# ChaissonLab/LRA

Measured on AMD Instinct MI355X. Metric: aligned Gbp/s, 30 kb ONT vs GRCh38 (MapRead_lowacc end to end incl. SAM text), per job, higher is better.
Workload: dtype int32

## Files before the change

### lra_amd/csrc/common.h

```cpp
#pragma once
#include <hip/hip_runtime.h>
#include <stdint.h>
#include <stdio.h>
#include <atomic>
#include <memory>
#include <string>
#include <string.h>
#include <vector>
#include "../../include/lra_hip.h"

struct lra_seed_state;
struct lra_cluster_state;
struct lra_map_state;
struct lra_handover;
void lra_handover_free(lra_ctx* ctx);
struct lra_gen_cell { std::atomic<uint64_t> gen{0}; std::atomic<bool> dead{false}; };
struct lra_time_rec { const char* name; hipEvent_t a, b; hipStream_t stream; };

struct lra_ctx {
  int device = 0;
  hipStream_t stream = nullptr;
  std::string err;
  void* scratch[4] = {nullptr, nullptr, nullptr, nullptr};
  size_t scratch_bytes[4] = {0, 0, 0, 0};
  int num_cu = 256;
  lra_seed_state* seed = nullptr;
  lra_cluster_state* clus = nullptr;
  lra_map_state* map = nullptr;
  void* aux = nullptr; size_t aux_bytes = 0;
  void* out_buf = nullptr; size_t out_bytes = 0;
  void* pin_buf = nullptr; size_t pin_bytes = 0;
  void* rec_pin = nullptr; size_t rec_pin_bytes = 0;
  void* sv_pin = nullptr; size_t sv_pin_bytes = 0;
  void* bgzf_pin = nullptr; size_t bgzf_pin_bytes = 0;
  std::vector<uint64_t> bgzf_member_off;
  int bgzf_round = 0;
  double bgzf_ms = 0; uint64_t bgzf_bytes = 0;
  void* bam_buf[6] = {}; size_t bam_bytes[6] = {};
  int bam_cigar_limit = 65535;
  uint64_t* scan_tmp = nullptr;
  static constexpr int N_SIDE = 4;
  hipStream_t side[N_SIDE] = {}; hipEvent_t ev_fork = nullptr, ev_join[N_SIDE] = {}, ev_mid = nullptr;
  void* gbuf[192] = {};
  size_t gbytes[192] = {};
  bool sdp_inner = false;
  bool timing = false;
  std::vector<lra_time_rec> recs;
  std::vector<hipEvent_t> free_events;
  lra_ctx* child = nullptr;
  bool owns_stream = false;
  bool pipelined = false;
  struct lra_handover* handover = nullptr;
  struct { bool valid = false; int n_reads = 0; const char* d_seq = nullptr; const uint64_t* d_read_off = nullptr; int k = 0, w = 0, max_freq = 0; lra_seed_result res; } ahead;
  bool store_all = false;
  int svsig_len = 25;
  bool low_priority = false; int prio = 0;
};

hipStream_t lra_side_fork(lra_ctx* ctx, int i = 0);
void lra_side_join(lra_ctx* ctx, int i = 0);
hipError_t lra_segsort_pairs(lra_ctx* ctx, void* temp, size_t& temp_bytes, const uint64_t* kin, uint64_t* kout, const uint32_t* vin, uint32_t* vout, unsigned int total,
                             unsigned int nseg, const uint64_t* b, const uint64_t* e, int begin_bit, int end_bit, hipStream_t st);
int lra_segsort_pairs_scratch(lra_ctx* ctx, const uint64_t* kin, uint64_t* kout, const uint32_t* vin, uint32_t* vout, uint64_t total, uint64_t nseg, const uint64_t* b,
                              const uint64_t* e, int begin_bit, int end_bit);
void lra_time_begin(lra_ctx* ctx, const char* name, hipStream_t stream = nullptr);
void lra_time_end(lra_ctx* ctx, hipStream_t stream = nullptr);
void lra_seed_free(lra_ctx* ctx);
void lra_cluster_free(lra_ctx* ctx);
void lra_map_free(lra_ctx* ctx);

int lra_set_err(lra_ctx* ctx, int code, const char* fmt, ...);
int lra_host_threads();
void* lra_scratch(lra_ctx* ctx, int slot, size_t bytes);
void* lra_pinned(lra_ctx* ctx, size_t bytes);
void* lra_ensure(lra_ctx* ctx, int idx, size_t bytes);

struct lra_sort_opts { const char* tag = "sort"; const char* fb_tag = "sort_fallback"; bool short_lists = false; };
int lra_sort_exact_batch(lra_ctx* ctx, int n_lists, const uint64_t* d_off, uint64_t* d_key, uint32_t* d_pos, const lra_sort_opts& o = lra_sort_opts(),
                         const int* only = nullptr);
int lra_sort_mostly_unique_batch(lra_ctx* ctx, int n_lists, const uint64_t* d_off, uint64_t total, uint64_t* d_key, uint32_t* d_pos,
                                 uint64_t* tmp_key, uint32_t* tmp_pos, int end_bit, const lra_sort_opts& o = lra_sort_opts());

int lra_launch_linear_extend(lra_ctx* ctx, uint64_t n_clusters, int K, const uint64_t* c_start, const uint64_t* c_end, const int* c_strand, const int* c_chrom,
                             int* c_read, const uint32_t* cl_q, const uint32_t* cl_t, const uint64_t* d_chrom_pos, const unsigned char* genome,
                             const unsigned char* seq, const uint64_t* read_off, uint32_t* e_q, uint32_t* e_t, int* e_len, uint32_t* e_count, uint32_t* box,
                             const int* c_K = nullptr);

int lra_format_bed_str(const lra_aln_record* r, std::string& s_);
int lra_format_paf_str(const lra_aln_record* r, int print_cigar, std::string& s_);
int lra_format_sam_str(const lra_aln_record* g, int n_group, int as, int hard_clip, const char* passthrough, std::string& s_);
int lra_format_sam_simple_str(const lra_aln_record* rp, int hard_clip, const char* passthrough, std::string& s_);
int lra_output_read_str(const lra_aln_group* groups, const int32_t* index, int n_groups, lra_aln_record* recs, int print_num_aln, char format, int hard_clip,
                        const char* passthrough, int read_unaligned, const lra_aln_record* unaligned_rec, std::string& text);

#define LRA_HIP_CHECK(ctx, call)                                                         \
  do {                                                                                   \
    hipError_t e__ = (call);                                                             \
    if (e__ != hipSuccess)                                                               \
      return lra_set_err(ctx, LRA_ERR_HIP, "%s failed: %s (%s:%d)", #call,               \
                         hipGetErrorString(e__), __FILE__, __LINE__);                    \
  } while (0)
```

### lra_amd/csrc/exact_sort.hip

```cpp
#include "common.h"
#include "kmer.h"
#include "std_sort.h"
#include <algorithm>

namespace {

constexpr int SORT_CAP = 9000;

struct MaskedLess {
  template <class V> __host__ __device__ __forceinline__ bool operator()(const V& a, const V& b) const { return (a.k & KM_FOR_MASK) < (b.k & KM_FOR_MASK); }
};

__global__ void __launch_bounds__(64) sort_kernel(int n_reads, const uint64_t* __restrict__ mm_off, uint64_t* mm_key, uint32_t* mm_pos,
                                                  const int* __restrict__ only_flagged) {
  const int r = blockIdx.x * 64 + threadIdx.x;
  if (r >= n_reads) return;
  if (only_flagged && !only_flagged[r]) return;
  lra_std_sort::std_sort(lra_std_sort::Pairs<uint32_t>{mm_key + mm_off[r], mm_pos + mm_off[r]}, (long)(mm_off[r + 1] - mm_off[r]), MaskedLess());
}

constexpr int SORT_NT = 1024;
constexpr int SORT_NW = SORT_NT / 64;

template <int MODE> struct SortTypes { typedef unsigned short IT; typedef uint32_t TT; };
template <> struct SortTypes<2> { typedef uint32_t IT; typedef uint64_t TT; };
__host__ __device__ inline size_t sort_scratch_bytes(int mode, size_t cap) {
  const size_t isz = mode == 2 ? 4 : 2, maxseg = (cap / 16 + 8 + 1) & ~(size_t)1;
  size_t b = cap * 8 + 4 * cap * isz + 64;
  if (mode == 2) b += 10 * maxseg * isz + (cap / 32 + 2) * 4 + 64;
  return (b + 255) & ~(size_t)255;
}
template <int MODE>
__global__ void __launch_bounds__(SORT_NT) sort_wg_kernel(int n_reads, const uint64_t* __restrict__ mm_off, uint64_t* mm_key, uint32_t* mm_pos,
                                                        void* tscratch, int cap, int* __restrict__ fallback,
                                                        const int* __restrict__ only, char* gscr, int* stat, int minLen = 0) {
  constexpr bool BIG = MODE >= 1, HUGE = MODE == 2;
  typedef typename SortTypes<MODE>::IT IT;
  typedef typename SortTypes<MODE>::TT TT;
  constexpr IT S_NONE = (IT)~(IT)0;
  constexpr int HB = HUGE ? 32 : 16;
  constexpr TT HM = (TT)(((TT)1 << HB) - 1);
  extern __shared__ __attribute__((aligned(16))) char smem[];
  const int tid = threadIdx.x, lane = tid & 63, wave = tid >> 6;
  const int NT_ = (int)blockDim.x, NW_ = NT_ >> 6;
  const int maxseg = (cap / 16 + 8 + 1) & ~1;
  char* ebase = BIG ? gscr + (size_t)blockIdx.x * sort_scratch_bytes(MODE, (size_t)cap) : smem;
  uint64_t* key = (uint64_t*)ebase;
  IT* idx = (IT*)(key + cap);
  IT* seg = idx + cap;
  IT* pa = seg + cap;
  IT* pb = pa + cap;
  IT* sF = HUGE ? pb + cap : BIG ? (IT*)smem : pb + cap;
  IT* sL = sF + maxseg;
  IT* sD = sL + maxseg;
  IT* nF = sD + maxseg;
  IT* nL = nF + maxseg;
  IT* nD = nL + maxseg;
  IT* sCut = nD + maxseg;
  IT* sLid = sCut + maxseg;
  IT* sRid = sLid + maxseg;
  IT* sM = sRid + maxseg;
  unsigned int* startBits = (unsigned int*)(sM + maxseg + (maxseg & 1));
  __shared__ int cnt[4];
  __shared__ unsigned int waveTot[2 * SORT_NW];
  TT* t32 = (TT*)tscratch + (size_t)blockIdx.x * (size_t)(cap + 64);
  const lra_std_sort::Pairs<IT> S{key, idx};
  const MaskedLess lt;
  for (int r = blockIdx.x; r < n_reads; r += gridDim.x) {
    const long base = (long)mm_off[r];
    const int n = (int)(mm_off[r + 1] - mm_off[r]);
    if (n < 2) continue;
    if (BIG) {
      if (!fallback[r]) continue;
      if (n > cap) { if (MODE == 1 && stat && tid == 0) { atomicMax(&stat[0], n); atomicAdd(&stat[1], 1); } continue; }
    } else {
      if (only && !only[r]) continue;
      if (n < minLen) continue;
      if (n > cap) { if (fallback && tid == 0) { fallback[r] = 1; if (stat) atomicAdd(&stat[2], 1); } continue; }
    }
    __syncthreads();
    if (BIG && tid == 0) fallback[r] = 0;
    for (int p = tid; p < n; p += NT_) { key[p] = mm_key[base + p]; idx[p] = (IT)p; seg[p] = 0; }
    for (int x = tid; x < cap / 32 + 1; x += NT_) startBits[x] = 0;
    if (tid == 0) {
      if (n > 16) { sF[0] = 0; sL[0] = (IT)n; sD[0] = (IT)(2 * (31 - __clz(n))); cnt[0] = 1; }
      else cnt[0] = 0;
      cnt[1] = 0;
    }
    __syncthreads();
    if (tid == 0) startBits[0] = 1u;
    int nseg = cnt[0];
    while (nseg > 0) {
      for (int s = tid; s < nseg; s += NT_) {
        const int first = (int)sF[s], last = (int)sL[s];
        sM[s] = 0;
        if (sD[s] == 0) { lra_std_sort::heap_sort(S, first, last, lt); sM[s] = S_NONE; continue; }
        sD[s] = sD[s] - 1;
        lra_std_sort::move_median_to_first(S, first, last, lt);
      }
      __syncthreads();
      const int rows = (n + 63) / 64, rpw = (rows + NW_ - 1) / NW_;
      const int r0 = wave * rpw, r1 = min(rows, r0 + rpw);
      auto flags = [&](int p, bool& A, bool& B) {
        A = false; B = false;
        if (p < n) {
          const IT sg = seg[p];
          if (sg != S_NONE && sM[sg] != S_NONE && p != (int)sF[sg]) {
            const uint64_t piv = key[sF[sg]] & KM_FOR_MASK, km = key[p] & KM_FOR_MASK;
            A = km >= piv; B = km <= piv;
          }
        }
      };
      unsigned int totA = 0, totB = 0;
      for (int rw = r0; rw < r1; rw++) {
        bool A, B; flags(rw * 64 + lane, A, B);
        totA += __popcll(__ballot(A)); totB += __popcll(__ballot(B));
      }
      if (lane == 0) { waveTot[wave] = totA; waveTot[NW_ + wave] = totB; }
      __syncthreads();
      unsigned int baseA = 0, baseB = 0;
      for (int w = 0; w < wave; w++) { baseA += waveTot[w]; baseB += waveTot[NW_ + w]; }
      const unsigned long long below = (lane == 0) ? 0ULL : (~0ULL >> (64 - lane));
      for (int rw = r0; rw < r1; rw++) {
        const int p = rw * 64 + lane;
        bool A, B; flags(p, A, B);
        const unsigned long long mA = __ballot(A), mB = __ballot(B);
        if (p <= n) t32[p] = ((TT)(baseA + __popcll(mA & below)) & HM) | ((TT)(baseB + __popcll(mB & below)) << HB);
        baseA += __popcll(mA); baseB += __popcll(mB);
      }
      if (wave == NW_ - 1 && lane == 0 && (n & 63) == 0) t32[n] = ((TT)baseA & HM) | ((TT)baseB << HB);
      __syncthreads();
      for (int p = tid; p < n; p += NT_) {
        bool A, B; flags(p, A, B);
        if (A || B) {
          const int sg = (int)seg[p], b0 = (int)sF[sg] + 1;
          const TT t = t32[p], tb = t32[b0], te = t32[sL[sg]];
          if (A) pa[b0 + (int)(((t & HM) - (tb & HM)) & HM)] = (IT)p;
          if (B) pb[b0 + (int)(((te >> HB) - (t >> HB) - 1) & HM)] = (IT)p;
        }
      }
      __syncthreads();
      for (int p = tid; p < n; p += NT_) {
        const IT sg = seg[p];
        if (sg == S_NONE || sM[sg] == S_NONE) continue;
        const int b0 = (int)sF[sg] + 1, i = p - b0;
        if (i < 0) continue;
        const TT tb = t32[b0], te = t32[sL[sg]];
        const int nA = (int)(((te & HM) - (tb & HM)) & HM), nB = (int)(((te >> HB) - (tb >> HB)) & HM);
        const int lim = min(nA, nB);
        if (i < lim && pa[b0 + i] < pb[b0 + i] && !(i + 1 < lim && pa[b0 + i + 1] < pb[b0 + i + 1])) sM[sg] = (IT)(i + 1);
      }
      __syncthreads();
      for (int p = tid; p < n; p += NT_) {
        const IT sg = seg[p];
        if (sg == S_NONE || sM[sg] == S_NONE) continue;
        const int b0 = (int)sF[sg] + 1, i = p - b0;
        if (i >= 0 && i < (int)sM[sg]) lra_std_sort::iter_swap(S, (int)pa[b0 + i], (int)pb[b0 + i]);
      }
      __syncthreads();
      for (int s = tid; s < nseg; s += NT_) {
        const int first = (int)sF[s], last = (int)sL[s];
        if (sM[s] == S_NONE) { sCut[s] = (IT)last; sLid[s] = S_NONE; sRid[s] = S_NONE; continue; }
        const int b0 = first + 1, m = (int)sM[s];
        const TT tb = t32[b0], te = t32[last];
        const int nA = (int)(((te & HM) - (tb & HM)) & HM);
        int cut = 0x7fffffff;
        if (m < nA) cut = pa[b0 + m];
        if (m >= 1) cut = min(cut, (int)pb[b0 + m - 1]);
        sCut[s] = (IT)cut;
        IT lid = S_NONE, rid = S_NONE;
        if (cut - first > 16) { int x = atomicAdd(&cnt[1], 1); nF[x] = (IT)first; nL[x] = (IT)cut; nD[x] = sD[s]; lid = (IT)x; }
        if (last - cut > 16) { int x = atomicAdd(&cnt[1], 1); nF[x] = (IT)cut; nL[x] = (IT)last; nD[x] = sD[s]; rid = (IT)x; }
        atomicOr(&startBits[cut >> 5], 1u << (cut & 31));
        sLid[s] = lid; sRid[s] = rid;
      }
      __syncthreads();
      for (int p = tid; p < n; p += NT_) {
        const IT sg = seg[p];
        if (sg != S_NONE) seg[p] = (p < (int)sCut[sg]) ? sLid[sg] : sRid[sg];
      }
      nseg = cnt[1];
      __syncthreads();
      for (int s = tid; s < nseg; s += NT_) { sF[s] = nF[s]; sL[s] = nL[s]; sD[s] = nD[s]; }
      if (tid == 0) cnt[1] = 0;
      __syncthreads();
    }
    for (int p = tid; p < n; p += NT_) {
      if ((startBits[p >> 5] >> (p & 31)) & 1u) {
        int q = p + 1;
        while (q < n && !((startBits[q >> 5] >> (q & 31)) & 1u)) q++;
        lra_std_sort::insertion_sort(S, p, q, lt);
      }
    }
    __syncthreads();
    uint32_t* tmp = HUGE ? (uint32_t*)seg : (uint32_t*)pa;
    for (int p = tid; p < n; p += NT_) tmp[p] = mm_pos[base + idx[p]];
    __syncthreads();
    for (int p = tid; p < n; p += NT_) { mm_key[base + p] = key[p]; mm_pos[base + p] = tmp[p]; }
  }
}

}

int lra_sort_exact_batch(lra_ctx* ctx, int n_reads, const uint64_t* mm_off, uint64_t* mm_key, uint32_t* mm_pos, const lra_sort_opts& o, const int* only) {
  hipStream_t st = ctx->stream;
  const int nb = (n_reads + 63) / 64;
  const int cap = SORT_CAP, capB = 65534;
  const int maxseg = (cap / 16 + 8 + 1) & ~1, maxsegB = (capB / 16 + 8 + 1) & ~1;
  const size_t lds = (size_t)cap * 16 + (size_t)maxseg * 20 + 8 + (size_t)(cap / 32 + 2) * 4;
  const size_t ldsB = (size_t)maxsegB * 20 + 8 + (size_t)(capB / 32 + 2) * 4 + 64;
  const int grid = n_reads < ctx->num_cu ? n_reads : ctx->num_cu;
  const int gridB = std::min(grid, 64);
  const size_t tszB = (size_t)gridB * (capB + 64) * 4, esz = (size_t)gridB * sort_scratch_bytes(1, (size_t)capB);
  uint32_t* tscr = (uint32_t*)lra_scratch(ctx, 0, (size_t)grid * (cap + 64) * 4 + (size_t)n_reads * 4);
  char* big = (char*)lra_ensure(ctx, 85, tszB + esz + 1024);
  int* stat = (int*)lra_ensure(ctx, 97, 64);
  if (!tscr || !big || !stat) return LRA_ERR_NOMEM;
  uint32_t* tscrB = (uint32_t*)big; char* gscr = big + tszB;
  int* flags = (int*)(tscr + (size_t)grid * (cap + 64));
  LRA_HIP_CHECK(ctx, hipMemsetAsync(flags, 0, (size_t)n_reads * 4, st));
  LRA_HIP_CHECK(ctx, hipMemsetAsync(stat, 0, 12, st));
  LRA_HIP_CHECK(ctx, hipFuncSetAttribute((const void*)sort_wg_kernel<0>, hipFuncAttributeMaxDynamicSharedMemorySize, (int)lds));
  LRA_HIP_CHECK(ctx, hipFuncSetAttribute((const void*)sort_wg_kernel<1>, hipFuncAttributeMaxDynamicSharedMemorySize, (int)ldsB));
  lra_time_begin(ctx, o.tag);
  constexpr int capS = 2048;
  if (o.short_lists) {
    const int maxsegS = (capS / 16 + 8 + 1) & ~1;
    const size_t ldsS = (size_t)capS * 16 + (size_t)maxsegS * 20 + 8 + (size_t)(capS / 32 + 2) * 4;
    const int gridS = std::min(n_reads, std::min(ctx->num_cu * 4, (int)(((size_t)grid * (cap + 64)) / (size_t)(capS + 64))));
    hipLaunchKernelGGL(sort_wg_kernel<0>, dim3(gridS), dim3(256), ldsS, st, n_reads, mm_off, mm_key, mm_pos, (void*)tscr, capS, (int*)nullptr, only, (char*)nullptr, (int*)nullptr, 0);
  }
  hipLaunchKernelGGL(sort_wg_kernel<0>, dim3(grid), dim3(SORT_NT), lds, st, n_reads, mm_off, mm_key, mm_pos, (void*)tscr, cap, flags, only, (char*)nullptr, stat, o.short_lists ? capS + 1 : 0);
  lra_time_end(ctx);
  int h_left = 1;
  LRA_HIP_CHECK(ctx, hipMemcpyAsync(&h_left, stat + 2, 4, hipMemcpyDeviceToHost, st));
  LRA_HIP_CHECK(ctx, hipStreamSynchronize(st));
  if (h_left == 0) return LRA_OK;
  lra_time_begin(ctx, o.tag);
  hipLaunchKernelGGL(sort_wg_kernel<1>, dim3(gridB), dim3(SORT_NT), ldsB, st, n_reads, mm_off, mm_key, mm_pos, (void*)tscrB, capB, flags, only, gscr, stat);
  lra_time_end(ctx);
  int h_stat[2] = {0, 0};
  LRA_HIP_CHECK(ctx, hipMemcpyAsync(h_stat, stat, 8, hipMemcpyDeviceToHost, st));
  LRA_HIP_CHECK(ctx, hipStreamSynchronize(st));
  if (h_stat[1] == 0) return LRA_OK;
  const int capH = std::min(h_stat[0] + 64, (1 << 26));
  const int gridH = std::min(h_stat[1], std::max(1, ctx->num_cu));
  const size_t eszH = sort_scratch_bytes(2, (size_t)capH), tszH = (size_t)(capH + 64) * 8;
  char* huge = (char*)lra_ensure(ctx, 98, (size_t)gridH * (eszH + tszH) + 1024);
  if (!huge) return LRA_ERR_NOMEM;
  lra_time_begin(ctx, o.tag);
  hipLaunchKernelGGL(sort_wg_kernel<2>, dim3(gridH), dim3(SORT_NT), 0, st, n_reads, mm_off, mm_key, mm_pos, (void*)huge, capH, flags, only, huge + (size_t)gridH * tszH, (int*)nullptr);
  lra_time_end(ctx);
  if (h_stat[0] > capH) {
    lra_time_begin(ctx, o.fb_tag);
    hipLaunchKernelGGL(sort_kernel, dim3(nb), dim3(64), 0, st, n_reads, mm_off, mm_key, mm_pos, (const int*)flags);
    lra_time_end(ctx);
  }
  return LRA_OK;
}

__global__ void __launch_bounds__(256) sort_adopt_kernel(int n_lists, const uint64_t* __restrict__ off, uint64_t* key, uint32_t* pos,
                                                         const uint64_t* __restrict__ tkey, const uint32_t* __restrict__ tpos, int* ties, int* n_ties) {
  const int r = blockIdx.x;
  const uint64_t b = off[r], e = off[r + 1];
  int tie = 0;
  for (uint64_t i = b + threadIdx.x; i + 1 < e; i += 256) tie |= (tkey[i] & KM_FOR_MASK) == (tkey[i + 1] & KM_FOR_MASK);
  tie = __syncthreads_or(tie);
  if (tie) { if (threadIdx.x == 0) { ties[r] = 1; atomicAdd(n_ties, 1); } return; }
  if (threadIdx.x == 0) ties[r] = 0;
  for (uint64_t i = b + threadIdx.x; i < e; i += 256) { key[i] = tkey[i]; pos[i] = tpos[i]; }
}

int lra_sort_mostly_unique_batch(lra_ctx* ctx, int n_lists, const uint64_t* d_off, uint64_t total, uint64_t* d_key, uint32_t* d_pos,
                                 uint64_t* tmp_key, uint32_t* tmp_pos, int end_bit, const lra_sort_opts& o) {
  if (n_lists == 0 || total == 0) return LRA_OK;
  hipStream_t st = ctx->stream;
  size_t temp_bytes = 0;
  (void)lra_segsort_pairs(ctx, nullptr, temp_bytes, nullptr, nullptr, nullptr, nullptr, (unsigned int)total, (unsigned int)n_lists, nullptr, nullptr, 0, end_bit, st);
  char* temp = (char*)lra_scratch(ctx, 2, temp_bytes + 512 + (size_t)n_lists * 4);
  if (!temp) return LRA_ERR_NOMEM;
  int* ties = (int*)(temp + ((temp_bytes + 255) & ~(size_t)255));
  int* n_ties = ties + n_lists + 1;
  LRA_HIP_CHECK(ctx, hipMemsetAsync(n_ties, 0, 4, st));
  lra_time_begin(ctx, o.tag);
  hipError_t e = lra_segsort_pairs(ctx, temp, temp_bytes, d_key, tmp_key, d_pos, tmp_pos, (unsigned int)total, (unsigned int)n_lists, d_off, d_off + 1, 0, end_bit, st);
  if (e != hipSuccess) { lra_time_end(ctx); return lra_set_err(ctx, LRA_ERR_HIP, "segmented sort: %s", hipGetErrorString(e)); }
  hipLaunchKernelGGL(sort_adopt_kernel, dim3(n_lists), dim3(256), 0, st, n_lists, d_off, d_key, d_pos, (const uint64_t*)tmp_key, (const uint32_t*)tmp_pos, ties, n_ties);
  lra_time_end(ctx);
  int h_ties = 1;
  LRA_HIP_CHECK(ctx, hipMemcpyAsync(&h_ties, n_ties, 4, hipMemcpyDeviceToHost, st));
  LRA_HIP_CHECK(ctx, hipStreamSynchronize(st));
  if (h_ties == 0) return LRA_OK;
  int rc = lra_sort_exact_batch(ctx, n_lists, d_off, d_key, d_pos, o, ties);
  if (rc) return rc;
  LRA_HIP_CHECK(ctx, hipGetLastError());
  return LRA_OK;
}

extern "C" int lra_sort_minimizers_batch(lra_ctx* ctx, int n_lists, const uint64_t* d_off, uint64_t* d_key, uint32_t* d_pos) {
  if (!ctx || n_lists < 0) return LRA_ERR_INVALID;
  if (n_lists == 0) return LRA_OK;
  LRA_HIP_CHECK(ctx, hipSetDevice(ctx->device));
  int rc = lra_sort_exact_batch(ctx, n_lists, d_off, d_key, d_pos);
  if (rc) return rc;
  LRA_HIP_CHECK(ctx, hipGetLastError());
  return LRA_OK;
}

extern "C" int lra_sort_minimizers_host(uint64_t n, uint64_t* h_key, uint32_t* h_pos) {
  if (n && (!h_key || !h_pos)) return LRA_ERR_INVALID;
  lra_std_sort::std_sort(lra_std_sort::Pairs<uint32_t>{h_key, h_pos}, (long)n, MaskedLess());
  return LRA_OK;
}
```

### lra_amd/csrc/refine_space.hip

```cpp
#include "common.h"
#include <stdlib.h>
#include "scan.h"
#include <algorithm>

int lra_aog_launch_device(lra_ctx* ctx, int n, const char* d_qseq, const char* d_tseq, const uint64_t* d_q_off, const int32_t* d_q_len,
                          const uint64_t* d_t_off, const int32_t* d_t_len, const int32_t* d_k, int m, int mm, int indel, int32_t* d_score,
                          int32_t* d_nblocks, int32_t* d_blocks, const uint64_t* d_block_off, int32_t* d_status);

namespace {

constexpr uint64_t FOR_MASK = 0x7FFFFFFFFFFFFFFFULL;
constexpr int MAX_W = 32;

__device__ __forceinline__ int code_n(unsigned char c) {
  if (c < 8) return c & 3;
  switch (c) { case 'A': case 'a': return 0; case 'C': case 'c': return 1; case 'G': case 'g': return 2; case 'T': case 't': return 3; default: return 4; }
}
__device__ __forceinline__ int code(unsigned char c) { const int v = code_n(c); return v > 3 ? 0 : v; }

struct RsArgs {
  int n;
  const char* qseq; const char* tseq; const uint64_t* q_off; const int32_t* q_len; const uint64_t* t_off; const int32_t* t_len;
  const uint32_t* t_span; const int32_t* K; const int32_t* W; const int32_t* diag; const uint32_t* q_add; const uint32_t* t_add; const uint32_t* flip;
  long maxFreq; const int32_t* maxFreqArr;
// ... 451 lines not shown
                             int mismatch, int indel, int max_freq, const int32_t* d_max_freq, lra_refine_space_result* out) {
  if (!ctx || !out || n < 0) return LRA_ERR_INVALID;
  memset(out, 0, sizeof *out);
  out->n_problems = (uint64_t)n;
  if (n == 0) return LRA_OK;
  LRA_HIP_CHECK(ctx, hipSetDevice(ctx->device));
  hipStream_t st = ctx->stream;
  const size_t n1 = (size_t)n + 2;
  auto take = [](char*& p, size_t cnt, size_t e) { char* r = p; p += sz(cnt, e); return r; };
  size_t needW = sz(n1, 4) * 8 + sz(n1, 8) * 6 + 2 * (sz(2 * n1, 4) + sz(2 * n1 + 2, 8)) + sz(4, 8) + 4096;
  char* w = (char*)lra_ensure(ctx, 14, needW);
  if (!w) return LRA_ERR_NOMEM;
  RsArgs a;
  memset(&a, 0, sizeof a);
  a.n = n; a.qseq = d_qseq; a.tseq = d_tseq; a.q_off = d_q_off; a.q_len = d_q_len; a.t_off = d_t_off; a.t_len = d_t_len; a.t_span = d_t_span; a.K = d_K; a.W = d_W;
  a.diag = d_diag; a.q_add = d_q_add; a.t_add = d_t_add; a.flip = d_flip_len; a.maxFreq = max_freq; a.maxFreqArr = d_max_freq;
  a.isSmall = (uint32_t*)take(w, n1, 4); a.smallIdx = (uint32_t*)take(w, n1, 4); a.largeIdx = (uint32_t*)take(w, n1, 4); a.sq_len = (int32_t*)take(w, n1, 4);
  a.st_len = (int32_t*)take(w, n1, 4); a.sk = (int32_t*)take(w, n1, 4); a.bcap = (uint32_t*)take(w, n1, 4); a.cnt = (uint32_t*)take(w, n1, 4);
  a.smallPos = (uint64_t*)take(w, n1, 8); a.sq_off = (uint64_t*)take(w, n1, 8); a.st_off = (uint64_t*)take(w, n1, 8);
  uint64_t* boff = (uint64_t*)take(w, n1, 8); uint64_t* pair_off = (uint64_t*)take(w, n1, 8); uint64_t* spare8 = (uint64_t*)take(w, n1, 8); (void)spare8;
  a.lcnt = (uint32_t*)take(w, 2 * n1, 4); uint64_t* loff = (uint64_t*)take(w, 2 * n1 + 2, 8);
  a.totals = (unsigned long long*)take(w, 4, 8);
  size_t needR = sz(n1, 8) + sz(n1, 4) * 2 + 4096;
  const unsigned g = (unsigned)((n + 255) / 256);
  float* identity; uint32_t* status; uint64_t* pairOffOut;
  {
    char* r0 = (char*)lra_ensure(ctx, 15, needR);
    if (!r0) return LRA_ERR_NOMEM;
    pairOffOut = (uint64_t*)take(r0, n1, 8); identity = (float*)take(r0, n1, 4); status = (uint32_t*)take(r0, n1, 4);
  }
  a.identity = identity; a.status = status;
  LRA_HIP_CHECK(ctx, hipMemsetAsync(a.totals, 0, 4 * 8, st));
  lra_time_begin(ctx, "refine_space");
  hipLaunchKernelGGL(rs_classify, dim3(g), dim3(256), 0, st, a);
  lra_time_end(ctx);
  unsigned long long totals[3] = {0, 0, 0};
  LRA_HIP_CHECK(ctx, hipMemcpyAsync(totals, a.totals, sizeof totals, hipMemcpyDeviceToHost, st));
  { int rc = lra_exclusive_scan<uint32_t>(ctx, n, a.isSmall, a.smallPos); if (rc) return rc; }
  LRA_HIP_CHECK(ctx, hipStreamSynchronize(st));
  const int nSmall = (int)totals[0], nLarge = n - nSmall;
  hipLaunchKernelGGL(rs_split, dim3(g), dim3(256), 0, st, a);
  int32_t* blocks = nullptr;
  if (nSmall > 0) {
    { int rc = lra_exclusive_scan<uint32_t>(ctx, nSmall, a.bcap, boff); if (rc) return rc; }
    const uint64_t totalCap = totals[1];
    size_t needB = sz(3 * totalCap + 3, 4) + sz((size_t)nSmall + 1, 4) * 3 + 4096;
    char* wb = (char*)lra_ensure(ctx, 16, needB);
    if (!wb) return LRA_ERR_NOMEM;
    blocks = (int32_t*)take(wb, 3 * totalCap + 3, 4);
    int32_t* score = (int32_t*)take(wb, (size_t)nSmall + 1, 4); int32_t* nblocks = (int32_t*)take(wb, (size_t)nSmall + 1, 4);
    int32_t* ast = (int32_t*)take(wb, (size_t)nSmall + 1, 4);
    int rc = lra_aog_launch_device(ctx, nSmall, d_qseq, d_tseq, a.sq_off, a.sq_len, a.st_off, a.st_len, a.sk, match, mismatch, indel, score, nblocks, blocks,
                                   boff, ast);
    if (rc) return rc;
    a.boff = boff; a.nblocks = nblocks; a.blocks = blocks; a.aogStatus = ast;
    lra_time_begin(ctx, "refine_space");
    hipLaunchKernelGGL(rs_small<false>, dim3((nSmall + 63) / 64), dim3(64), 0, st, a, nSmall);
    lra_time_end(ctx);
  }
  if (nLarge > 0) {
    uint32_t* lcap = (uint32_t*)take(w, 2 * n1, 4); uint64_t* capOff = (uint64_t*)take(w, 2 * n1 + 2, 8);
    hipLaunchKernelGGL(rs_caps, dim3((2 * nLarge + 255) / 256), dim3(256), 0, st, a, nLarge, lcap);
    { int rc = lra_exclusive_scan<uint32_t>(ctx, 2 * nLarge, lcap, capOff); if (rc) return rc; }
    const uint64_t totalCap = totals[2];
    char* wr = (char*)lra_ensure(ctx, 66, sz(totalCap + 1, 8) + sz(totalCap + 1, 4) + 4096);
    if (!wr) return LRA_ERR_NOMEM;
    uint64_t* rawKey = (uint64_t*)take(wr, totalCap + 1, 8); uint32_t* rawPos = (uint32_t*)take(wr, totalCap + 1, 4);
    a.lkey = rawKey; a.lpos = rawPos; a.loff = capOff;
    lra_time_begin(ctx, "rs_long_sketch");
    hipLaunchKernelGGL(rs_sketch<true>, dim3(2 * nLarge), dim3(64), 0, st, a, nLarge);
    lra_time_end(ctx);
    { int rc = lra_exclusive_scan<uint32_t>(ctx, 2 * nLarge, a.lcnt, loff); if (rc) return rc; }
    uint64_t totalMm = 0;
    LRA_HIP_CHECK(ctx, hipMemcpyAsync(&totalMm, loff + 2 * nLarge, 8, hipMemcpyDeviceToHost, st));
    LRA_HIP_CHECK(ctx, hipStreamSynchronize(st));
    if (getenv("LRA_RS_DBG")) fprintf(stderr, "[rs] n %d nLarge %d minimizers %llu\n", n, nLarge, (unsigned long long)totalMm);
    char* wl = (char*)lra_ensure(ctx, 17, sz(totalMm + 1, 8) + sz(totalMm + 1, 4) + sz(totalMm + 2 * (size_t)nLarge + 4, 16) + sz((size_t)nLarge + 1, 4) +
                                          sz(totalMm + 1, 16) + 4096);
    if (!wl) return LRA_ERR_NOMEM;
    a.lkey = (uint64_t*)take(wl, totalMm + 1, 8); a.lpos = (uint32_t*)take(wl, totalMm + 1, 4); a.loff = loff;
    a.rects = (int4*)take(wl, totalMm + 2 * (size_t)nLarge + 4, 16); a.nrect = (uint32_t*)take(wl, (size_t)nLarge + 1, 4);
    a.tab = (uint4*)take(wl, totalMm + 1, 16);
    hipLaunchKernelGGL(rs_compact, dim3(2 * nLarge), dim3(64), 0, st, 2 * nLarge, capOff, loff, rawKey, rawPos, a.lkey, a.lpos);
    { int rc = lra_sort_minimizers_batch(ctx, 2 * nLarge, loff, a.lkey, a.lpos); if (rc) return rc; }
    lra_time_begin(ctx, "rs_long_compare");
    hipLaunchKernelGGL(rs_bounds, dim3(2 * nLarge), dim3(256), 0, st, a, nLarge);
    hipLaunchKernelGGL(rs_compare, dim3(nLarge), dim3(64), 0, st, a, nLarge);
    hipLaunchKernelGGL(rs_count, dim3(nLarge), dim3(64), 0, st, a, nLarge);
    lra_time_end(ctx);
  }
  { int rc = lra_exclusive_scan<uint32_t>(ctx, n, a.cnt, pair_off); if (rc) return rc; }
  uint64_t nPairs = 0;
  LRA_HIP_CHECK(ctx, hipMemcpyAsync(&nPairs, pair_off + n, 8, hipMemcpyDeviceToHost, st));
  LRA_HIP_CHECK(ctx, hipStreamSynchronize(st));
  char* r = (char*)lra_ensure(ctx, 11, sz(nPairs + 1, 4) * 2 + 4096);
  if (!r) return LRA_ERR_NOMEM;
  uint32_t* outQ = (uint32_t*)take(r, nPairs + 1, 4); uint32_t* outT = (uint32_t*)take(r, nPairs + 1, 4);
  LRA_HIP_CHECK(ctx, hipMemcpyAsync(pairOffOut, pair_off, ((size_t)n + 1) * 8, hipMemcpyDeviceToDevice, st));
  a.pair_off = pairOffOut; a.outQ = outQ; a.outT = outT;
  lra_time_begin(ctx, "refine_space");
  if (nSmall > 0) hipLaunchKernelGGL(rs_small<true>, dim3((nSmall + 63) / 64), dim3(64), 0, st, a, nSmall);
  lra_time_end(ctx);
  if (nLarge > 0) {
    lra_time_begin(ctx, "rs_long_compare");
    hipLaunchKernelGGL(rs_emit, dim3(nLarge), dim3(64), 0, st, a, nLarge);
    lra_time_end(ctx);
  }
  LRA_HIP_CHECK(ctx, hipStreamSynchronize(st));
  LRA_HIP_CHECK(ctx, hipGetLastError());
  out->n_pairs = nPairs; out->n_small = (uint64_t)nSmall; out->d_pair_off = pairOffOut; out->d_pair_q = outQ; out->d_pair_t = outT; out->d_identity = identity;
  out->d_status = status;
  return LRA_OK;
}

extern "C" int lra_refine_space_batch(lra_ctx* ctx, int n, const char* d_qseq, const uint64_t* d_q_off, const int32_t* d_q_len, const char* d_tseq,
                                      const uint64_t* d_t_off, const int32_t* d_t_len, const uint32_t* d_t_span, const int32_t* d_K, const int32_t* d_W,
                                      const int32_t* d_diag, const uint32_t* d_q_add, const uint32_t* d_t_add, const uint32_t* d_flip_len, int match,
                                      int mismatch, int indel, int max_freq, lra_refine_space_result* out) {
  return refine_space_impl(ctx, n, d_qseq, d_q_off, d_q_len, d_tseq, d_t_off, d_t_len, d_t_span, d_K, d_W, d_diag, d_q_add, d_t_add, d_flip_len, match, mismatch,
                           indel, max_freq, nullptr, out);
}

extern "C" int lra_refine_space_batch_mf(lra_ctx* ctx, int n, const char* d_qseq, const uint64_t* d_q_off, const int32_t* d_q_len, const char* d_tseq,
                                         const uint64_t* d_t_off, const int32_t* d_t_len, const uint32_t* d_t_span, const int32_t* d_K, const int32_t* d_W,
                                         const int32_t* d_diag, const uint32_t* d_q_add, const uint32_t* d_t_add, const uint32_t* d_flip_len, int match,
                                         int mismatch, int indel, const int32_t* d_max_freq, lra_refine_space_result* out) {
  if (!d_max_freq) return LRA_ERR_INVALID;
  return refine_space_impl(ctx, n, d_qseq, d_q_off, d_q_len, d_tseq, d_t_off, d_t_len, d_t_span, d_K, d_W, d_diag, d_q_add, d_t_add, d_flip_len, match, mismatch,
                           indel, 0, d_max_freq, out);
}
```

Before: 1.151.

## Reuse radix-sorted keys to restrict exact tie-breaking sort to tied runs

The exact std::sort-equivalent workgroup sort now takes the radix-sorted keys as a hint. It records which masked keys have duplicate runs, builds a small LDS table of tie groups, and keeps partitioning only on rows that still hold tied elements, tracked through an active-row list. Elements with unique keys are written straight from the radix result, and tied ones are scattered into their run positions. Minimizer sorts (generic and refine_space long reads) now go through the radix-first mostly-unique path, and a count of large tied lists is passed along so the host no longer needs a sync before the big-mode kernel. This adds complexity and new LDS layout risk for equivalence with the original sort order.

```diff
diff --git a/lra_amd/csrc/common.h b/lra_amd/csrc/common.h
--- a/lra_amd/csrc/common.h
+++ b/lra_amd/csrc/common.h
@@ -77,7 +77,8 @@
 
 struct lra_sort_opts { const char* tag = "sort"; const char* fb_tag = "sort_fallback"; bool short_lists = false; };
 int lra_sort_exact_batch(lra_ctx* ctx, int n_lists, const uint64_t* d_off, uint64_t* d_key, uint32_t* d_pos, const lra_sort_opts& o = lra_sort_opts(),
-                         const int* only = nullptr);
+                         const int* only = nullptr,
+                         const uint64_t* sorted_key = nullptr, const uint32_t* sorted_pos = nullptr, int n_large = -1);
 int lra_sort_mostly_unique_batch(lra_ctx* ctx, int n_lists, const uint64_t* d_off, uint64_t total, uint64_t* d_key, uint32_t* d_pos,
                                  uint64_t* tmp_key, uint32_t* tmp_pos, int end_bit, const lra_sort_opts& o = lra_sort_opts());
 
diff --git a/lra_amd/csrc/exact_sort.hip b/lra_amd/csrc/exact_sort.hip
--- a/lra_amd/csrc/exact_sort.hip
+++ b/lra_amd/csrc/exact_sort.hip
@@ -6,6 +6,7 @@
 namespace {
 
 constexpr int SORT_CAP = 9000;
+constexpr int SORT_GCAP = 128;
 
 struct MaskedLess {
   template <class V> __host__ __device__ __forceinline__ bool operator()(const V& a, const V& b) const { return (a.k & KM_FOR_MASK) < (b.k & KM_FOR_MASK); }
@@ -30,14 +31,21 @@
   if (mode == 2) b += 10 * maxseg * isz + (cap / 32 + 2) * 4 + 64;
   return (b + 255) & ~(size_t)255;
 }
+inline size_t sort_lds_bytes(int mode, size_t cap, size_t gcap) {
+  if (mode == 2) return 0;
+  const size_t maxseg = (cap / 16 + 8 + 1) & ~(size_t)1, W = cap / 32 + 2;
+  return (mode == 0 ? cap * 16 : 0) + maxseg * 20 + gcap * 8 + (3 * W + maxseg + 32) * 4 + (gcap + cap / 64 + 2) * 2 + 16;
+}
 template <int MODE>
 __global__ void __launch_bounds__(SORT_NT) sort_wg_kernel(int n_reads, const uint64_t* __restrict__ mm_off, uint64_t* mm_key, uint32_t* mm_pos,
                                                         void* tscratch, int cap, int* __restrict__ fallback,
-                                                        const int* __restrict__ only, char* gscr, int* stat, int minLen = 0) {
+                                                        const int* __restrict__ only, char* gscr, int* stat, int minLen = 0,
+                                                        const uint64_t* tkey = nullptr, const uint32_t* tpos = nullptr, int gcap = 0) {
   constexpr bool BIG = MODE >= 1, HUGE = MODE == 2;
   typedef typename SortTypes<MODE>::IT IT;
   typedef typename SortTypes<MODE>::TT TT;
   constexpr IT S_NONE = (IT)~(IT)0;
+  constexpr IT S_CT = (IT)(S_NONE - 1);
   constexpr int HB = HUGE ? 32 : 16;
   constexpr TT HM = (TT)(((TT)1 << HB) - 1);
   extern __shared__ __attribute__((aligned(16))) char smem[];
@@ -60,12 +68,21 @@
   IT* sLid = sCut + maxseg;
   IT* sRid = sLid + maxseg;
   IT* sM = sRid + maxseg;
-  unsigned int* startBits = (unsigned int*)(sM + maxseg + (maxseg & 1));
+  const int W = cap / 32 + 2;
+  uint64_t* tk = (uint64_t*)(sM + maxseg);
+  unsigned int* startBits = HUGE ? (unsigned int*)(sM + maxseg + (maxseg & 1)) : (unsigned int*)(tk + gcap);
+  unsigned int* sortBits = HUGE ? startBits : startBits + W;
+  unsigned int* tiedBits = sortBits + W;
+  unsigned int* cntLR = tiedBits + W;
+  unsigned int* rowBits = cntLR + maxseg;
+  IT* rb = (IT*)(rowBits + 32);
+  IT* actRow = rb + gcap;
   __shared__ int cnt[4];
   __shared__ unsigned int waveTot[2 * SORT_NW];
   TT* t32 = (TT*)tscratch + (size_t)blockIdx.x * (size_t)(cap + 64);
   const lra_std_sort::Pairs<IT> S{key, idx};
   const MaskedLess lt;
+  const unsigned long long below = (lane == 0) ? 0ULL : (~0ULL >> (64 - lane));
   for (int r = blockIdx.x; r < n_reads; r += gridDim.x) {
     const long base = (long)mm_off[r];
     const int n = (int)(mm_off[r + 1] - mm_off[r]);
@@ -81,15 +98,74 @@
     __syncthreads();
     if (BIG && tid == 0) fallback[r] = 0;
     for (int p = tid; p < n; p += NT_) { key[p] = mm_key[base + p]; idx[p] = (IT)p; seg[p] = 0; }
-    for (int x = tid; x < cap / 32 + 1; x += NT_) startBits[x] = 0;
+    for (int x = tid; x < cap / 32 + 1; x += NT_) { startBits[x] = 0; if (!HUGE) sortBits[x] = 0; }
+    const int rows = (n + 63) / 64;
+    bool allOpen = HUGE || tkey == nullptr;
+    int G = 0;
+    if (!HUGE && tkey != nullptr) {
+      const uint64_t* tkl = tkey + base;
+      const int rpw = (rows + NW_ - 1) / NW_, r0 = wave * rpw, r1 = min(rows, r0 + rpw);
+      int bad = 0;
+      auto runStart = [&](int j, uint64_t& km) {
+        if (j >= n) return false;
+        km = tkl[j] & KM_FOR_MASK;
+        const bool eqPrev = j > 0 && (tkl[j - 1] & KM_FOR_MASK) == km, eqNext = j + 1 < n && (tkl[j + 1] & KM_FOR_MASK) == km;
+        if (j > 0 && (tkl[j - 1] & KM_FOR_MASK) > km) bad = 1;
+        return eqNext && !eqPrev;
+      };
+      unsigned int tot = 0;
+      for (int rw = r0; rw < r1; rw++) { uint64_t km; tot += __popcll(__ballot(runStart(rw * 64 + lane, km))); }
+      if (lane == 0) waveTot[wave] = tot;
+      bad = __syncthreads_or(bad);
+      int g0 = 0;
+      for (int w = 0; w < NW_; w++) { if (w < wave) g0 += (int)waveTot[w]; G += (int)waveTot[w]; }
+      if (bad || G > gcap) allOpen = true;
+      if (!allOpen) {
+        for (int rw = r0; rw < r1; rw++) {
+          const int j = rw * 64 + lane;
+          uint64_t km = 0;
+          const bool f = runStart(j, km);
+          const unsigned long long m = __ballot(f);
+          if (f) { const int g = g0 + __popcll(m & below); tk[g] = km; rb[g] = (IT)j; }
+          g0 += __popcll(m);
+        }
+      }
+      __syncthreads();
+    }
+    auto lookup = [&](uint64_t km) {
+      int lo = 0, hi = G;
+      while (lo < hi) { const int mid = (lo + hi) >> 1; if (tk[mid] < km) lo = mid + 1; else hi = mid; }
+      return (lo < G && tk[lo] == km) ? lo : -1;
+    };
+    if (!HUGE && !allOpen)
+      for (int rw = wave; rw < rows; rw += NW_) {
+        const int p = rw * 64 + lane;
+        const unsigned long long m = __ballot(p < n && lookup(key[p] & KM_FOR_MASK) >= 0);
+        if (lane == 0) { tiedBits[2 * rw] = (unsigned int)m; tiedBits[2 * rw + 1] = (unsigned int)(m >> 32); }
+      }
+    auto tied = [&](int x) { return allOpen || ((tiedBits[x >> 5] >> (x & 31)) & 1u); };
+    if (!HUGE) { for (int a = tid; a < rows; a += NT_) actRow[a] = (IT)a; if (tid < 32) rowBits[tid] = 0; }
+    const bool rootOpen = allOpen || G > 0;
     if (tid == 0) {
-      if (n > 16) { sF[0] = 0; sL[0] = (IT)n; sD[0] = (IT)(2 * (31 - __clz(n))); cnt[0] = 1; }
+      if (n > 16 && rootOpen) { sF[0] = 0; sL[0] = (IT)n; sD[0] = (IT)(2 * (31 - __clz(n))); cnt[0] = 1; }
       else cnt[0] = 0;
-      cnt[1] = 0;
+      cnt[1] = 0; cnt[2] = rows;
     }
     __syncthreads();
-    if (tid == 0) startBits[0] = 1u;
-    int nseg = cnt[0];
+    if (tid == 0) { startBits[0] = 1u; if (n <= 16 && rootOpen) sortBits[0] |= 1u; }
+    int nseg = cnt[0], nAct = rows;
+    auto rowAt = [&](int a) { return HUGE ? a : (int)actRow[a]; };
+    auto makeChildren = [&](int s, int cL, int cR) {
+      const int first = (int)sF[s], last = (int)sL[s], cut = (int)sCut[s];
+      IT lid = S_NONE, rid = S_NONE;
+      if (cL < 2) lid = S_CT;
+      else if (cut - first > 16) { int x = atomicAdd(&cnt[1], 1); nF[x] = (IT)first; nL[x] = (IT)cut; nD[x] = sD[s]; lid = (IT)x; }
+      else atomicOr(&sortBits[first >> 5], 1u << (first & 31));
+      if (cR < 2) rid = S_CT;
+      else if (last - cut > 16) { int x = atomicAdd(&cnt[1], 1); nF[x] = (IT)cut; nL[x] = (IT)last; nD[x] = sD[s]; rid = (IT)x; }
+      else atomicOr(&sortBits[cut >> 5], 1u << (cut & 31));
+      sLid[s] = lid; sRid[s] = rid;
+    };
     while (nseg > 0) {
       for (int s = tid; s < nseg; s += NT_) {
         const int first = (int)sF[s], last = (int)sL[s];
@@ -99,13 +175,13 @@
         lra_std_sort::move_median_to_first(S, first, last, lt);
       }
       __syncthreads();
-      const int rows = (n + 63) / 64, rpw = (rows + NW_ - 1) / NW_;
-      const int r0 = wave * rpw, r1 = min(rows, r0 + rpw);
+      const int rpw = (nAct + NW_ - 1) / NW_;
+      const int r0 = wave * rpw, r1 = min(nAct, r0 + rpw);
       auto flags = [&](int p, bool& A, bool& B) {
         A = false; B = false;
         if (p < n) {
           const IT sg = seg[p];
-          if (sg != S_NONE && sM[sg] != S_NONE && p != (int)sF[sg]) {
+          if (sg < S_CT && sM[sg] != S_NONE && p != (int)sF[sg]) {
             const uint64_t piv = key[sF[sg]] & KM_FOR_MASK, km = key[p] & KM_FOR_MASK;
             A = km >= piv; B = km <= piv;
           }
@@ -113,102 +189,162 @@
       };
       unsigned int totA = 0, totB = 0;
       for (int rw = r0; rw < r1; rw++) {
-        bool A, B; flags(rw * 64 + lane, A, B);
+        bool A, B; flags(rowAt(rw) * 64 + lane, A, B);
         totA += __popcll(__ballot(A)); totB += __popcll(__ballot(B));
       }
       if (lane == 0) { waveTot[wave] = totA; waveTot[NW_ + wave] = totB; }
       __syncthreads();
       unsigned int baseA = 0, baseB = 0;
       for (int w = 0; w < wave; w++) { baseA += waveTot[w]; baseB += waveTot[NW_ + w]; }
-      const unsigned long long below = (lane == 0) ? 0ULL : (~0ULL >> (64 - lane));
       for (int rw = r0; rw < r1; rw++) {
-        const int p = rw * 64 + lane;
+        const int p = rowAt(rw) * 64 + lane;
         bool A, B; flags(p, A, B);
         const unsigned long long mA = __ballot(A), mB = __ballot(B);
-        if (p <= n) t32[p] = ((TT)(baseA + __popcll(mA & below)) & HM) | ((TT)(baseB + __popcll(mB & below)) << HB);
+        if (p < n) t32[p] = ((TT)(baseA + __popcll(mA & below) + (A ? 1 : 0)) & HM) | ((TT)(baseB + __popcll(mB & below) + (B ? 1 : 0)) << HB);
         baseA += __popcll(mA); baseB += __popcll(mB);
       }
-      if (wave == NW_ - 1 && lane == 0 && (n & 63) == 0) t32[n] = ((TT)baseA & HM) | ((TT)baseB << HB);
-      __syncthreads();
-      for (int p = tid; p < n; p += NT_) {
+      __syncthreads();
+      for (int a = wave; a < nAct; a += NW_) {
+        const int p = rowAt(a) * 64 + lane;
         bool A, B; flags(p, A, B);
         if (A || B) {
           const int sg = (int)seg[p], b0 = (int)sF[sg] + 1;
-          const TT t = t32[p], tb = t32[b0], te = t32[sL[sg]];
-          if (A) pa[b0 + (int)(((t & HM) - (tb & HM)) & HM)] = (IT)p;
-          if (B) pb[b0 + (int)(((te >> HB) - (t >> HB) - 1) & HM)] = (IT)p;
+          const TT t = t32[p], tb = t32[b0 - 1], te = t32[sL[sg] - 1];
+          if (A) pa[b0 + (int)(((t & HM) - 1 - (tb & HM)) & HM)] = (IT)p;
+          if (B) pb[b0 + (int)(((te >> HB) - (t >> HB)) & HM)] = (IT)p;
         }
       }
       __syncthreads();
-      for (int p = tid; p < n; p += NT_) {
+      for (int a = wave; a < nAct; a += NW_) {
+        const int p = rowAt(a) * 64 + lane;
+        if (p >= n) continue;
         const IT sg = seg[p];
-        if (sg == S_NONE || sM[sg] == S_NONE) continue;
+        if (sg >= S_CT || sM[sg] == S_NONE) continue;
         const int b0 = (int)sF[sg] + 1, i = p - b0;
         if (i < 0) continue;
-        const TT tb = t32[b0], te = t32[sL[sg]];
+        const TT tb = t32[b0 - 1], te = t32[sL[sg] - 1];
         const int nA = (int)(((te & HM) - (tb & HM)) & HM), nB = (int)(((te >> HB) - (tb >> HB)) & HM);
         const int lim = min(nA, nB);
         if (i < lim && pa[b0 + i] < pb[b0 + i] && !(i + 1 < lim && pa[b0 + i + 1] < pb[b0 + i + 1])) sM[sg] = (IT)(i + 1);
       }
       __syncthreads();
-      for (int p = tid; p < n; p += NT_) {
+      for (int a = wave; a < nAct; a += NW_) {
+        const int p = rowAt(a) * 64 + lane;
+        if (p >= n) continue;
         const IT sg = seg[p];
-        if (sg == S_NONE || sM[sg] == S_NONE) continue;
+        if (sg >= S_CT || sM[sg] == S_NONE) continue;
         const int b0 = (int)sF[sg] + 1, i = p - b0;
         if (i >= 0 && i < (int)sM[sg]) lra_std_sort::iter_swap(S, (int)pa[b0 + i], (int)pb[b0 + i]);
       }
       __syncthreads();
       for (int s = tid; s < nseg; s += NT_) {
         const int first = (int)sF[s], last = (int)sL[s];
+        if (!HUGE) cntLR[s] = 0;
         if (sM[s] == S_NONE) { sCut[s] = (IT)last; sLid[s] = S_NONE; sRid[s] = S_NONE; continue; }
         const int b0 = first + 1, m = (int)sM[s];
-        const TT tb = t32[b0], te = t32[last];
+        const TT tb = t32[first], te = t32[last - 1];
         const int nA = (int)(((te & HM) - (tb & HM)) & HM);
         int cut = 0x7fffffff;
         if (m < nA) cut = pa[b0 + m];
         if (m >= 1) cut = min(cut, (int)pb[b0 + m - 1]);
         sCut[s] = (IT)cut;
-        IT lid = S_NONE, rid = S_NONE;
-        if (cut - first > 16) { int x = atomicAdd(&cnt[1], 1); nF[x] = (IT)first; nL[x] = (IT)cut; nD[x] = sD[s]; lid = (IT)x; }
-        if (last - cut > 16) { int x = atomicAdd(&cnt[1], 1); nF[x] = (IT)cut; nL[x] = (IT)last; nD[x] = sD[s]; rid = (IT)x; }
         atomicOr(&startBits[cut >> 5], 1u << (cut & 31));
-        sLid[s] = lid; sRid[s] = rid;
-      }
-      __syncthreads();
-      for (int p = tid; p < n; p += NT_) {
-        const IT sg = seg[p];
-        if (sg != S_NONE) seg[p] = (p < (int)sCut[sg]) ? sLid[sg] : sRid[sg];
+        if (allOpen) makeChildren(s, 2, 2);
+      }
+      if (!HUGE && tid < 32) rowBits[tid] = 0;
+      __syncthreads();
+      if (!HUGE && !allOpen) {
+        for (int a = wave; a < nAct; a += NW_) {
+          const int p = rowAt(a) * 64 + lane;
+          bool part = false; unsigned int v = 0;
+          if (p < n) {
+            const IT sg = seg[p];
+            if (sg < S_CT && sM[sg] != S_NONE && tied((int)idx[p])) { part = true; v = ((unsigned int)sg << 1) | (p >= (int)sCut[sg] ? 1u : 0u); }
+          }
+          const unsigned long long m = __ballot(part);
+          if (m) {
+            const int leader = __ffsll((long long)m) - 1;
+            const unsigned int v0 = (unsigned int)__shfl((int)v, leader);
+            if (__ballot(part && v != v0) == 0) { if (lane == leader) atomicAdd(&cntLR[v0 >> 1], (unsigned int)__popcll(m) << ((v0 & 1u) * 16)); }
+            else if (part) atomicAdd(&cntLR[v >> 1], 1u << ((v & 1u) * 16));
+          }
+        }
+        __syncthreads();
+        for (int s = tid; s < nseg; s += NT_)
+          if (sM[s] != S_NONE) makeChildren(s, (int)(cntLR[s] & 0xffffu), (int)(cntLR[s] >> 16));
+        __syncthreads();
+      }
+      for (int a = wave; a < nAct; a += NW_) {
+        const int row = rowAt(a), p = row * 64 + lane;
+        IT nl = S_NONE;
+        if (p < n) {
+          const IT sg = seg[p];
+          if (sg < S_CT) {
+            if (sM[sg] != S_NONE) {
+              const bool right = p >= (int)sCut[sg];
+              nl = right ? sRid[sg] : sLid[sg];
+              if (nl == S_CT) {
+                if (tied((int)idx[p])) { const int g = lookup(key[p] & KM_FOR_MASK); pa[p] = (IT)max(right ? (int)sCut[sg] : (int)sF[sg], (int)rb[g]); }
+                else nl = S_NONE;
+              }
+            }
+            seg[p] = nl;
+          }
+        }
+        if (!HUGE) { const unsigned long long any = __ballot(nl < S_CT); if (lane == 0 && any) atomicOr(&rowBits[row >> 5], 1u << (row & 31)); }
       }
       nseg = cnt[1];
       __syncthreads();
       for (int s = tid; s < nseg; s += NT_) { sF[s] = nF[s]; sL[s] = nL[s]; sD[s] = nD[s]; }
       if (tid == 0) cnt[1] = 0;
-      __syncthreads();
+      if (!HUGE && wave == 0) {
+        unsigned int w = lane < 32 ? rowBits[lane] : 0u;
+        const int c = __popc(w);
+        int ex = c;
+        for (int d = 1; d < 64; d <<= 1) { const int t = __shfl_up(ex, d); if (lane >= d) ex += t; }
+        const int total = __shfl(ex, 63);
+        ex -= c;
+        while (w) { const int b = __ffs((int)w) - 1; w &= w - 1; actRow[ex++] = (IT)(lane * 32 + b); }
+        if (lane == 0) cnt[2] = total;
+      }
+      __syncthreads();
+      if (!HUGE) nAct = cnt[2];
     }
     for (int p = tid; p < n; p += NT_) {
-      if ((startBits[p >> 5] >> (p & 31)) & 1u) {
+      if ((sortBits[p >> 5] >> (p & 31)) & 1u) {
         int q = p + 1;
         while (q < n && !((startBits[q >> 5] >> (q & 31)) & 1u)) q++;
         lra_std_sort::insertion_sort(S, p, q, lt);
       }
     }
     __syncthreads();
-    uint32_t* tmp = HUGE ? (uint32_t*)seg : (uint32_t*)pa;
-    for (int p = tid; p < n; p += NT_) tmp[p] = mm_pos[base + idx[p]];
-    __syncthreads();
-    for (int p = tid; p < n; p += NT_) { mm_key[base + p] = key[p]; mm_pos[base + p] = tmp[p]; }
+    uint32_t* tmp = HUGE ? (uint32_t*)seg : allOpen ? (uint32_t*)pa : (uint32_t*)t32;
+    if (allOpen) {
+      for (int p = tid; p < n; p += NT_) tmp[p] = mm_pos[base + idx[p]];
+      __syncthreads();
+      for (int p = tid; p < n; p += NT_) { mm_key[base + p] = key[p]; mm_pos[base + p] = tmp[p]; }
+    } else {
+      for (int p = tid; p < n; p += NT_) if (tied((int)idx[p])) tmp[p] = mm_pos[base + idx[p]];
+      __syncthreads();
+      const uint64_t* tkl = tkey + base;
+      for (int p = tid; p < n; p += NT_) {
+        const uint64_t k = tkl[p], km = k & KM_FOR_MASK;
+        if (!((p > 0 && (tkl[p - 1] & KM_FOR_MASK) == km) || (p + 1 < n && (tkl[p + 1] & KM_FOR_MASK) == km))) { mm_key[base + p] = k; mm_pos[base + p] = tpos[base + p]; }
+        if (tied((int)idx[p])) { const int d = seg[p] == S_CT ? (int)pa[p] : p; mm_key[base + d] = key[p]; mm_pos[base + d] = tmp[p]; }
+      }
+    }
   }
 }
 
 }
 
-int lra_sort_exact_batch(lra_ctx* ctx, int n_reads, const uint64_t* mm_off, uint64_t* mm_key, uint32_t* mm_pos, const lra_sort_opts& o, const int* only) {
+int lra_sort_exact_batch(lra_ctx* ctx, int n_reads, const uint64_t* mm_off, uint64_t* mm_key, uint32_t* mm_pos, const lra_sort_opts& o, const int* only,
+                         const uint64_t* sorted_key, const uint32_t* sorted_pos, int n_large) {
   hipStream_t st = ctx->stream;
   const int nb = (n_reads + 63) / 64;
   const int cap = SORT_CAP, capB = 65534;
-  const int maxseg = (cap / 16 + 8 + 1) & ~1, maxsegB = (capB / 16 + 8 + 1) & ~1;
-  const size_t lds = (size_t)cap * 16 + (size_t)maxseg * 20 + 8 + (size_t)(cap / 32 + 2) * 4;
-  const size_t ldsB = (size_t)maxsegB * 20 + 8 + (size_t)(capB / 32 + 2) * 4 + 64;
+  const int gcap = SORT_GCAP, gcapB = 1024;
+  const size_t lds = sort_lds_bytes(0, cap, gcap), ldsB = sort_lds_bytes(1, capB, gcapB);
   const int grid = n_reads < ctx->num_cu ? n_reads : ctx->num_cu;
   const int gridB = std::min(grid, 64);
   const size_t tszB = (size_t)gridB * (capB + 64) * 4, esz = (size_t)gridB * sort_scratch_bytes(1, (size_t)capB);
@@ -225,19 +361,22 @@
   lra_time_begin(ctx, o.tag);
   constexpr int capS = 2048;
   if (o.short_lists) {
-    const int maxsegS = (capS / 16 + 8 + 1) & ~1;
-    const size_t ldsS = (size_t)capS * 16 + (size_t)maxsegS * 20 + 8 + (size_t)(capS / 32 + 2) * 4;
+    const size_t ldsS = sort_lds_bytes(0, capS, gcap);
     const int gridS = std::min(n_reads, std::min(ctx->num_cu * 4, (int)(((size_t)grid * (cap + 64)) / (size_t)(capS + 64))));
-    hipLaunchKernelGGL(sort_wg_kernel<0>, dim3(gridS), dim3(256), ldsS, st, n_reads, mm_off, mm_key, mm_pos, (void*)tscr, capS, (int*)nullptr, only, (char*)nullptr, (int*)nullptr, 0);
+    hipLaunchKernelGGL(sort_wg_kernel<0>, dim3(gridS), dim3(256), ldsS, st, n_reads, mm_off, mm_key, mm_pos, (void*)tscr, capS, (int*)nullptr, only, (char*)nullptr, (int*)nullptr, 0,
+                       sorted_key, sorted_pos, gcap);
   }
-  hipLaunchKernelGGL(sort_wg_kernel<0>, dim3(grid), dim3(SORT_NT), lds, st, n_reads, mm_off, mm_key, mm_pos, (void*)tscr, cap, flags, only, (char*)nullptr, stat, o.short_lists ? capS + 1 : 0);
+  hipLaunchKernelGGL(sort_wg_kernel<0>, dim3(grid), dim3(SORT_NT), lds, st, n_reads, mm_off, mm_key, mm_pos, (void*)tscr, cap, flags, only, (char*)nullptr, stat, o.short_lists ? capS + 1 : 0,
+                     sorted_key, sorted_pos, gcap);
   lra_time_end(ctx);
-  int h_left = 1;
-  LRA_HIP_CHECK(ctx, hipMemcpyAsync(&h_left, stat + 2, 4, hipMemcpyDeviceToHost, st));
-  LRA_HIP_CHECK(ctx, hipStreamSynchronize(st));
+  int h_left = n_large;
+  if (h_left < 0) {
+    LRA_HIP_CHECK(ctx, hipMemcpyAsync(&h_left, stat + 2, 4, hipMemcpyDeviceToHost, st));
+    LRA_HIP_CHECK(ctx, hipStreamSynchronize(st));
+  }
   if (h_left == 0) return LRA_OK;
   lra_time_begin(ctx, o.tag);
-  hipLaunchKernelGGL(sort_wg_kernel<1>, dim3(gridB), dim3(SORT_NT), ldsB, st, n_reads, mm_off, mm_key, mm_pos, (void*)tscrB, capB, flags, only, gscr, stat);
+  hipLaunchKernelGGL(sort_wg_kernel<1>, dim3(gridB), dim3(SORT_NT), ldsB, st, n_reads, mm_off, mm_key, mm_pos, (void*)tscrB, capB, flags, only, gscr, stat, 0, sorted_key, sorted_pos, gcapB);
   lra_time_end(ctx);
   int h_stat[2] = {0, 0};
   LRA_HIP_CHECK(ctx, hipMemcpyAsync(h_stat, stat, 8, hipMemcpyDeviceToHost, st));
@@ -266,7 +405,7 @@
   int tie = 0;
   for (uint64_t i = b + threadIdx.x; i + 1 < e; i += 256) tie |= (tkey[i] & KM_FOR_MASK) == (tkey[i + 1] & KM_FOR_MASK);
   tie = __syncthreads_or(tie);
-  if (tie) { if (threadIdx.x == 0) { ties[r] = 1; atomicAdd(n_ties, 1); } return; }
+  if (tie) { if (threadIdx.x == 0) { ties[r] = 1; atomicAdd(n_ties, 1); if (e - b > (uint64_t)SORT_CAP) atomicAdd(n_ties + 1, 1); } return; }
   if (threadIdx.x == 0) ties[r] = 0;
   for (uint64_t i = b + threadIdx.x; i < e; i += 256) { key[i] = tkey[i]; pos[i] = tpos[i]; }
 }
@@ -277,21 +416,26 @@
   hipStream_t st = ctx->stream;
   size_t temp_bytes = 0;
   (void)lra_segsort_pairs(ctx, nullptr, temp_bytes, nullptr, nullptr, nullptr, nullptr, (unsigned int)total, (unsigned int)n_lists, nullptr, nullptr, 0, end_bit, st);
-  char* temp = (char*)lra_scratch(ctx, 2, temp_bytes + 512 + (size_t)n_lists * 4);
+  const size_t flag_bytes = (512 + (size_t)n_lists * 4 + 255) & ~(size_t)255;
+  char* temp = (char*)lra_scratch(ctx, 2, temp_bytes + flag_bytes + (tmp_key ? 0 : ((size_t)total * 12 + 512)));
   if (!temp) return LRA_ERR_NOMEM;
   int* ties = (int*)(temp + ((temp_bytes + 255) & ~(size_t)255));
   int* n_ties = ties + n_lists + 1;
-  LRA_HIP_CHECK(ctx, hipMemsetAsync(n_ties, 0, 4, st));
+  if (!tmp_key) {
+    tmp_key = (uint64_t*)((char*)ties + flag_bytes);
+    tmp_pos = (uint32_t*)(tmp_key + total + 1);
+  }
+  LRA_HIP_CHECK(ctx, hipMemsetAsync(n_ties, 0, 8, st));
   lra_time_begin(ctx, o.tag);
   hipError_t e = lra_segsort_pairs(ctx, temp, temp_bytes, d_key, tmp_key, d_pos, tmp_pos, (unsigned int)total, (unsigned int)n_lists, d_off, d_off + 1, 0, end_bit, st);
   if (e != hipSuccess) { lra_time_end(ctx); return lra_set_err(ctx, LRA_ERR_HIP, "segmented sort: %s", hipGetErrorString(e)); }
   hipLaunchKernelGGL(sort_adopt_kernel, dim3(n_lists), dim3(256), 0, st, n_lists, d_off, d_key, d_pos, (const uint64_t*)tmp_key, (const uint32_t*)tmp_pos, ties, n_ties);
   lra_time_end(ctx);
-  int h_ties = 1;
-  LRA_HIP_CHECK(ctx, hipMemcpyAsync(&h_ties, n_ties, 4, hipMemcpyDeviceToHost, st));
+  int h_ties[2] = {1, 1};
+  LRA_HIP_CHECK(ctx, hipMemcpyAsync(h_ties, n_ties, 8, hipMemcpyDeviceToHost, st));
   LRA_HIP_CHECK(ctx, hipStreamSynchronize(st));
-  if (h_ties == 0) return LRA_OK;
-  int rc = lra_sort_exact_batch(ctx, n_lists, d_off, d_key, d_pos, o, ties);
+  if (h_ties[0] == 0) return LRA_OK;
+  int rc = lra_sort_exact_batch(ctx, n_lists, d_off, d_key, d_pos, o, ties, tmp_key, tmp_pos, h_ties[1]);
   if (rc) return rc;
   LRA_HIP_CHECK(ctx, hipGetLastError());
   return LRA_OK;
@@ -301,7 +445,11 @@
   if (!ctx || n_lists < 0) return LRA_ERR_INVALID;
   if (n_lists == 0) return LRA_OK;
   LRA_HIP_CHECK(ctx, hipSetDevice(ctx->device));
-  int rc = lra_sort_exact_batch(ctx, n_lists, d_off, d_key, d_pos);
+  uint64_t total = 0;
+  LRA_HIP_CHECK(ctx, hipMemcpyAsync(&total, d_off + n_lists, 8, hipMemcpyDeviceToHost, ctx->stream));
+  LRA_HIP_CHECK(ctx, hipStreamSynchronize(ctx->stream));
+  int rc = total >> 32 ? lra_sort_exact_batch(ctx, n_lists, d_off, d_key, d_pos)
+                       : lra_sort_mostly_unique_batch(ctx, n_lists, d_off, total, d_key, d_pos, nullptr, nullptr, 63);
   if (rc) return rc;
   LRA_HIP_CHECK(ctx, hipGetLastError());
   return LRA_OK;
diff --git a/lra_amd/csrc/refine_space.hip b/lra_amd/csrc/refine_space.hip
--- a/lra_amd/csrc/refine_space.hip
+++ b/lra_amd/csrc/refine_space.hip
@@ -557,7 +557,7 @@
     a.rects = (int4*)take(wl, totalMm + 2 * (size_t)nLarge + 4, 16); a.nrect = (uint32_t*)take(wl, (size_t)nLarge + 1, 4);
     a.tab = (uint4*)take(wl, totalMm + 1, 16);
     hipLaunchKernelGGL(rs_compact, dim3(2 * nLarge), dim3(64), 0, st, 2 * nLarge, capOff, loff, rawKey, rawPos, a.lkey, a.lpos);
-    { int rc = lra_sort_minimizers_batch(ctx, 2 * nLarge, loff, a.lkey, a.lpos); if (rc) return rc; }
+    { int rc = lra_sort_mostly_unique_batch(ctx, 2 * nLarge, loff, totalMm, a.lkey, a.lpos, nullptr, nullptr, 63); if (rc) return rc; }
     lra_time_begin(ctx, "rs_long_compare");
     hipLaunchKernelGGL(rs_bounds, dim3(2 * nLarge), dim3(256), 0, st, a, nLarge);
     hipLaunchKernelGGL(rs_compare, dim3(nLarge), dim3(64), 0, st, a, nLarge);
```

Result: slower. 1.130 (-1.9%).
